# thu-nics/Rad-NeRF

Measured on AMD Instinct MI355X. Metric: million samples/s fwd+bwd, 8192 rays, model_zoo_size=2; rgb L∞ vs ref, higher is better.
Workload: dtype f16/f32

## Files before the change

rad-nerf_amd/csrc/rn_march.h:

```cpp
#pragma once
#include "rn_common.h"
#pragma clang fp contract(off)

namespace {

struct MarchCfg {
    int cascades;
    int grid_size;
    int max_samples;
    float scale;
    float dt_scale;
    float esf;
    int abl;
};

struct NoSink {
    __device__ __forceinline__ void emit(int, float, float, float, float, float) const {}
};

struct RefSink {
    float* __restrict__ xyzs; float* __restrict__ dirs;
    float* __restrict__ ts;   float* __restrict__ deltas;
    float dx, dy, dz;
    __device__ __forceinline__ void emit(int s, float x, float y, float z, float t, float dt) const {
        xyzs[3 * s + 0] = x; xyzs[3 * s + 1] = y; xyzs[3 * s + 2] = z;
        dirs[3 * s + 0] = dx; dirs[3 * s + 1] = dy; dirs[3 * s + 2] = dz;
        ts[s] = t; deltas[s] = dt;
    }
};

struct StageSink {
    float* __restrict__ ts; float* __restrict__ deltas;
    __device__ __forceinline__ void emit(int s, float, float, float, float t, float dt) const {
        ts[s] = t; deltas[s] = dt;
    }
};

struct CompactSink {
    float* __restrict__ ts; float* __restrict__ deltas; int32_t* __restrict__ ray_of;
    int ray;
    __device__ __forceinline__ void emit(int s, float, float, float, float t, float dt) const {
        ts[s] = t; deltas[s] = dt; ray_of[s] = ray;
    }
};

__device__ __forceinline__ float mip_bound_inv(int mip, float scale) {
    return scalbnf(1.0f, mip - 1) < scale ? scalbnf(1.0f, 1 - mip) : 1.0f / scale;
}

__device__ __forceinline__ bool march_step(float& t, float ox, float oy, float oz,
                                           float dx, float dy, float dz,
                                           float dxi, float dyi, float dzi,
                                           const uint8_t* __restrict__ bitfield,
                                           const MarchCfg& c, float& x, float& y,
                                           float& z, float& dt) {
    const uint32_t g3 = (uint32_t)c.grid_size * c.grid_size * c.grid_size;
    const float gsi = 1.0f / c.grid_size;
    x = fmaf(t, dx, ox); y = fmaf(t, dy, oy); z = fmaf(t, dz, oz);
    dt = rn_calc_dt(t, c.esf, c.max_samples, c.grid_size, c.dt_scale);
    const int mip = max(rn_mip_from_pos(x, y, z, c.cascades),
                        rn_mip_from_dt(dt, c.grid_size, c.cascades));
    const float mb = fminf(scalbnf(1.0f, mip - 1), c.scale);
    const float mbi = mip_bound_inv(mip, c.scale);
    const float gm1 = c.grid_size - 1.0f;
    const int nx = (int)rn_clampf(0.5f * fmaf(x, mbi, 1.0f) * c.grid_size, 0.0f, gm1);
    const int ny = (int)rn_clampf(0.5f * fmaf(y, mbi, 1.0f) * c.grid_size, 0.0f, gm1);
    const int nz = (int)rn_clampf(0.5f * fmaf(z, mbi, 1.0f) * c.grid_size, 0.0f, gm1);
    const uint32_t idx = mip * g3 + rn_morton3d(nx, ny, nz);
    const bool occ = bitfield[idx / 8] & (1 << (idx % 8));
    if (occ) return true;
    const float tx = fmaf(fmaf(fmaf(0.5f, rn_signf(dx), nx + 0.5f) * gsi, 2.0f, -1.0f), mb, -x) * dxi;
    const float ty = fmaf(fmaf(fmaf(0.5f, rn_signf(dy), ny + 0.5f) * gsi, 2.0f, -1.0f), mb, -y) * dyi;
    const float tz = fmaf(fmaf(fmaf(0.5f, rn_signf(dz), nz + 0.5f) * gsi, 2.0f, -1.0f), mb, -z) * dzi;
    const float t_target = t + fmaxf(0.0f, fminf(tx, fminf(ty, tz)));
    do {
        t += rn_calc_dt(t, c.esf, c.max_samples, c.grid_size, c.dt_scale);
    } while (t < t_target);
    return false;
}

__device__ __forceinline__ bool march_query(float t, float ox, float oy, float oz,
                                            float dx, float dy, float dz,
                                            float dxi, float dyi, float dzi,
                                            const uint8_t* __restrict__ bitfield,
                                            const MarchCfg& c, float& x, float& y, float& z,
                                            float& dt, float& t_target) {
    const uint32_t g3 = (uint32_t)c.grid_size * c.grid_size * c.grid_size;
    const float gsi = 1.0f / c.grid_size;
    x = fmaf(t, dx, ox); y = fmaf(t, dy, oy); z = fmaf(t, dz, oz);
    dt = rn_calc_dt(t, c.esf, c.max_samples, c.grid_size, c.dt_scale);
    const int mip = max(rn_mip_from_pos(x, y, z, c.cascades),
                        rn_mip_from_dt(dt, c.grid_size, c.cascades));
    const float mb = fminf(scalbnf(1.0f, mip - 1), c.scale);
    const float mbi = mip_bound_inv(mip, c.scale);
    const float gm1 = c.grid_size - 1.0f;
    const int nx = (int)rn_clampf(0.5f * fmaf(x, mbi, 1.0f) * c.grid_size, 0.0f, gm1);
    const int ny = (int)rn_clampf(0.5f * fmaf(y, mbi, 1.0f) * c.grid_size, 0.0f, gm1);
    const int nz = (int)rn_clampf(0.5f * fmaf(z, mbi, 1.0f) * c.grid_size, 0.0f, gm1);
    const uint32_t idx = mip * g3 + rn_morton3d(nx, ny, nz);
    const bool occ = bitfield[idx / 8] & (1 << (idx % 8));
    const float tx = fmaf(fmaf(fmaf(0.5f, rn_signf(dx), nx + 0.5f) * gsi, 2.0f, -1.0f), mb, -x) * dxi;
    const float ty = fmaf(fmaf(fmaf(0.5f, rn_signf(dy), ny + 0.5f) * gsi, 2.0f, -1.0f), mb, -y) * dyi;
    const float tz = fmaf(fmaf(fmaf(0.5f, rn_signf(dz), nz + 0.5f) * gsi, 2.0f, -1.0f), mb, -z) * dzi;
    t_target = t + fmaxf(0.0f, fminf(tx, fminf(ty, tz)));
    return occ;
}

template <bool WRITE, typename Sink, bool NEG = false>
__device__ int march_ray_wave(float ox, float oy, float oz, float dx, float dy, float dz,
                              float t1, float t2, int cap, int start,
                              const uint8_t* __restrict__ bitfield, const MarchCfg& c,
                              const Sink& sink) {
    const int lane = rn_lane();
    if (!((NEG || 0.0f <= t1) && t1 < t2) || cap <= 0) return 0;
    const float dxi = 1.0f / dx, dyi = 1.0f / dy, dzi = 1.0f / dz;
    const uint64_t lt_mask = (1ull << lane) - 1ull;
    float tb = t1;
    float need = -INFINITY;
    int n = 0;
    int chunks = 0;
    while (true) {
        if (NEG && ++chunks > (1 << 16)) break;
        float t = tb;
        if (c.esf == 0.0f) {
            const float d0 = rn_calc_dt(0.0f, c.esf, c.max_samples, c.grid_size, c.dt_scale);
            const float s1 = tb + d0, r = s1 - tb, s2 = s1 + d0;
            const float bend = __uint_as_float((__float_as_uint(tb) & 0x7f800000u) + 0x00800000u);
            const float tj = fmaf((float)lane, r, tb);
            if (s2 - s1 == r && tb > 0.0f && __builtin_amdgcn_ballot_w64(!(tj < bend)) == 0) {
                t = tj;
            } else {
#pragma unroll 16
                for (int i = 0; i < RN_WAVE - 1; ++i) { const float nt = t + d0; t = i < lane ? nt : t; }
            }
        } else if (rn_dbg(c.abl) & 1) {
            t = fmaf((float)lane, rn_calc_dt(tb, c.esf, c.max_samples, c.grid_size, c.dt_scale), tb);
        } else {
#pragma unroll 8
            for (int i = 0; i < RN_WAVE - 1; ++i) {
                const float nt = t + rn_calc_dt(t, c.esf, c.max_samples, c.grid_size, c.dt_scale);
                t = i < lane ? nt : t;
            }
        }
        const bool alive = t < t2;
        float x, y, z, dt, target;
        const bool occ = march_query(t, ox, oy, oz, dx, dy, dz, dxi, dyi, dzi, bitfield, c,
                                     x, y, z, dt, target) && alive;
        const uint64_t alive_m = __builtin_amdgcn_ballot_w64(alive);
        const uint64_t occ_m = __builtin_amdgcn_ballot_w64(occ);
        uint64_t mark = 0;
        const uint64_t cand = __builtin_amdgcn_ballot_w64(alive && t >= need);
        int cur = cand ? __builtin_ctzll(cand) : RN_WAVE;
        int emitted = 0;
        bool full = false;
        const bool capfree = n + RN_WAVE < cap;
        while (cur < RN_WAVE) {
            const uint64_t from = ~0ull << cur;
            if ((occ_m >> cur) & 1ull) {
                const uint64_t stop = ~occ_m & from;
                const int end = stop ? __builtin_ctzll(stop) : RN_WAVE;
                need = -INFINITY;
                if (!capfree && n + emitted + (end - cur) >= cap) {
                    const int e2 = cur + (cap - n - emitted);
                    mark |= from & (e2 < RN_WAVE ? ~(~0ull << e2) : ~0ull);
                    emitted += e2 - cur;
                    full = true;
                    break;
                }
                mark |= from & ((stop & (0ull - stop)) - 1ull);
                emitted += end - cur;
                cur = (end < RN_WAVE && ((alive_m >> end) & 1ull)) ? end : RN_WAVE;
            } else {
                mark |= 1ull << cur;
                need = __int_as_float(__builtin_amdgcn_readlane(__float_as_int(target), cur));
                const uint64_t nxt = __builtin_amdgcn_ballot_w64(alive && t >= need) & (from << 1);
                cur = nxt ? __builtin_ctzll(nxt) : RN_WAVE;
            }
        }
        const uint64_t emit_m = mark & occ_m;
        if (WRITE && ((emit_m >> lane) & 1ull))
            sink.emit(start + n + __builtin_popcountll(emit_m & lt_mask), x, y, z, t, dt);
        n += __builtin_popcountll(emit_m);
        if (full || alive_m != ~0ull) break;
        const float tl = __int_as_float(__builtin_amdgcn_readlane(__float_as_int(t), RN_WAVE - 1));
        tb = tl + rn_calc_dt(tl, c.esf, c.max_samples, c.grid_size, c.dt_scale);
        if (!(tb < t2)) break;
    }
    return n;
}

__device__ __forceinline__ void aabb(float ox, float oy, float oz, float dx, float dy, float dz,
                                     const float* __restrict__ c, const float* __restrict__ h,
                                     float& t1, float& t2) {
    const float ix = 1.0f / dx, iy = 1.0f / dy, iz = 1.0f / dz;
    const float ax = (c[0] - h[0] - ox) * ix, bx = (c[0] + h[0] - ox) * ix;
    const float ay = (c[1] - h[1] - oy) * iy, by = (c[1] + h[1] - oy) * iy;
    const float az = (c[2] - h[2] - oz) * iz, bz = (c[2] + h[2] - oz) * iz;
    const float n = fmaxf(fmaxf(fminf(ax, bx), fminf(ay, by)), fminf(az, bz));
    const float f = fminf(fminf(fmaxf(ax, bx), fmaxf(ay, by)), fmaxf(az, bz));
    if (n > f) { t1 = -1.0f; t2 = -1.0f; } else { t1 = n; t2 = f; }
}

}
```

Baseline: 1197.

## Precompute per-lane skip links and walk them with readlane in ray march

```diff
diff --git a/rad-nerf_amd/csrc/rn_march.h b/rad-nerf_amd/csrc/rn_march.h
--- a/rad-nerf_amd/csrc/rn_march.h
+++ b/rad-nerf_amd/csrc/rn_march.h
@@ -148,39 +148,43 @@
                                      x, y, z, dt, target) && alive;
         const uint64_t alive_m = __builtin_amdgcn_ballot_w64(alive);
         const uint64_t occ_m = __builtin_amdgcn_ballot_w64(occ);
-        uint64_t mark = 0;
+        const uint64_t stop = ~occ_m & ~lt_mask;
+        const uint64_t run = ((stop & (0ull - stop)) - 1ull) & ~lt_mask;
+        const int end = stop ? __builtin_ctzll(stop) : RN_WAVE;
+        const int key = __float_as_int(alive ? t : INFINITY);
+        int lb = 0;
+#pragma unroll
+        for (int h = RN_WAVE / 2; h > 0; h >>= 1) {
+            const float kv = __int_as_float(__builtin_amdgcn_ds_bpermute((lb + h - 1) << 2, key));
+            lb += kv >= target ? 0 : h;
+        }
+        const float klast = __int_as_float(__builtin_amdgcn_readlane(key, RN_WAVE - 1));
+        lb += (lb == RN_WAVE - 1 && !(klast >= target)) ? 1 : 0;
+        const int to = occ ? end : max(lb, lane + 1);
+        const int link = (to < RN_WAVE && ((alive_m >> (to & (RN_WAVE - 1))) & 1ull)) ? to : RN_WAVE;
+        const uint64_t span = occ ? run : 1ull << lane;
+        const int span_lo = (int)(uint32_t)span, span_hi = (int)(uint32_t)(span >> 32);
         const uint64_t cand = __builtin_amdgcn_ballot_w64(alive && t >= need);
         int cur = cand ? __builtin_ctzll(cand) : RN_WAVE;
-        int emitted = 0;
-        bool full = false;
-        const bool capfree = n + RN_WAVE < cap;
+        int last = -1;
+        uint32_t mark_lo = 0, mark_hi = 0;
         while (cur < RN_WAVE) {
-            const uint64_t from = ~0ull << cur;
-            if ((occ_m >> cur) & 1ull) {
-                const uint64_t stop = ~occ_m & from;
-                const int end = stop ? __builtin_ctzll(stop) : RN_WAVE;
-                need = -INFINITY;
-                if (!capfree && n + emitted + (end - cur) >= cap) {
-                    const int e2 = cur + (cap - n - emitted);
-                    mark |= from & (e2 < RN_WAVE ? ~(~0ull << e2) : ~0ull);
-                    emitted += e2 - cur;
-                    full = true;
-                    break;
-                }
-                mark |= from & ((stop & (0ull - stop)) - 1ull);
-                emitted += end - cur;
-                cur = (end < RN_WAVE && ((alive_m >> end) & 1ull)) ? end : RN_WAVE;
-            } else {
-                mark |= 1ull << cur;
-                need = __int_as_float(__builtin_amdgcn_readlane(__float_as_int(target), cur));
-                const uint64_t nxt = __builtin_amdgcn_ballot_w64(alive && t >= need) & (from << 1);
-                cur = nxt ? __builtin_ctzll(nxt) : RN_WAVE;
-            }
+            mark_lo |= (uint32_t)__builtin_amdgcn_readlane(span_lo, cur);
+            mark_hi |= (uint32_t)__builtin_amdgcn_readlane(span_hi, cur);
+            last = cur;
+            cur = __builtin_amdgcn_readlane(link, cur);
         }
-        const uint64_t emit_m = mark & occ_m;
-        if (WRITE && ((emit_m >> lane) & 1ull))
-            sink.emit(start + n + __builtin_popcountll(emit_m & lt_mask), x, y, z, t, dt);
-        n += __builtin_popcountll(emit_m);
+        if (last >= 0)
+            need = ((occ_m >> last) & 1ull)
+                       ? -INFINITY
+                       : __int_as_float(__builtin_amdgcn_readlane(__float_as_int(target), last));
+        const uint64_t emit_m = ((uint64_t)mark_hi << 32 | mark_lo) & occ_m;
+        const int room = cap - n, found = __builtin_popcountll(emit_m);
+        const int before = __builtin_popcountll(emit_m & lt_mask);
+        const bool full = found >= room;
+        if (WRITE && ((emit_m >> lane) & 1ull) && before < room)
+            sink.emit(start + n + before, x, y, z, t, dt);
+        n += min(found, room);
         if (full || alive_m != ~0ull) break;
         const float tl = __int_as_float(__builtin_amdgcn_readlane(__float_as_int(t), RN_WAVE - 1));
         tb = tl + rn_calc_dt(tl, c.esf, c.max_samples, c.grid_size, c.dt_scale);
```

Result: faster. 1216, median of 6 (+1.6%).
